# Ipsedo/MARLClassification

Hardware: AMD Instinct MI355X
Metric: agent-env-steps/sec (higher is better)
Workload: dtype f32; 1 GPU; RESISC45 256x256x3, 16 agents, 16 steps, f=12, README dims (configs[2]); full train iteration: rollout + A2C loss + BPTT backward + Adam; batch_per_gpu=256, global_batch=256, parallelism=dp1, rng=library (Philox4x32-10), launch=eager

## Files before the change

marlclassification_amd/csrc/common.h:

```cpp
#pragma once

#include <hip/hip_runtime.h>
#include <stdint.h>
#include <stdio.h>

#include "../../include/marl_hip.h"
#include "../../include/marl_hip_gemmops.h"
#include "split.h"

namespace marl {

constexpr int kWave = 64;

inline int p4(int x) { return (x + 3) & ~3; }
inline int64_t cdiv(int64_t a, int64_t b) { return (a + b - 1) / b; }

void set_error(const char* fmt, ...);

int tune_get(const char* key, int dflt);
int tune_set(const char* key, int value);

__device__ __forceinline__ float rcp_fast(float x) { return __builtin_amdgcn_rcpf(x); }
__device__ __forceinline__ float sigmoid_acc(float x) { return rcp_fast(1.0f + __expf(-x)); }
__device__ __forceinline__ float tanh_fast(float x) { return 1.0f - 2.0f * rcp_fast(1.0f + __expf(2.0f * x)); }
// ... 72 lines not shown
};

constexpr int kMaxGemmBatch = 4;
struct GemmBatch {
    GemmProb p[kMaxGemmBatch];
    int count;
    int gx, gy;
    int xcd_map;
    int single_buf;
#ifdef MARL_KERNEL_TS
    long long* ts;
#endif
};

__device__ __forceinline__ void xcd_tile(unsigned gx, unsigned gy, unsigned gz, unsigned& bx,
                                         unsigned& by, unsigned& bz) {
    const unsigned T = gx * gy * gz, L = blockIdx.x;
    const unsigned per = T >> 3, rem = T & 7, xcd = L & 7, slot = L >> 3;
    const unsigned q = (xcd < rem ? xcd * (per + 1) : rem * (per + 1) + (xcd - rem) * per) + slot;
    bz = q / (gx * gy);
    const unsigned r = q - bz * gx * gy;
    bx = r / gy;
    by = r - bx * gy;
}

inline hipError_t raise_lds(const void* kern, size_t bytes) {
    static const void* done[128];
    static int ndone = 0;
    for (int i = 0; i < ndone; ++i)
        if (done[i] == kern) return hipSuccess;
    const hipError_t e = hipFuncSetAttribute(kern, hipFuncAttributeMaxDynamicSharedMemorySize, (int)bytes);
    if (e == hipSuccess && ndone < 128) done[ndone++] = kern;
    return e;
}

GemmProb gemm_prob(const float* a, int lda, const GemmB& b, float* c, int ldc, int m, int n,
                   const float* bias = nullptr, int accumulate = 0);
void gemm_add_seg(GemmProb& p, const float* a, int lda, const GemmB& b);

using GemmPlan = marl_gemm_plan_info;
inline dim3 plan_grid(const GemmPlan& p) { return p.xcd_map ? dim3(p.gx * p.gy * p.gz) : dim3(p.gx, p.gy, p.gz); }
GemmPlan gemm_nt_plan(const GemmBatch& batch);
GemmPlan gemm_lstm_plan(const GemmBatch& batch);
int launch_gemm_nt(const GemmBatch& batch, hipStream_t st);
int launch_gemm_lstm(const GemmBatch& batch, hipStream_t st);

int split_mode();
constexpr int kSplitRowBytes = 80;
size_t split_image_floats(int rows, int k);
struct SplitDesc {
    const float* src;
    void* dst;
    int rows, k, ld, kt;
};
constexpr int kMaxSplitDesc = 64;
struct SplitBatch {
    SplitDesc d[kMaxSplitDesc];
    int count;
};
int launch_split_weights(const SplitBatch& b, hipStream_t st);
int launch_gemm_nt_split(const GemmBatch& batch, const GemmPlan& plan, bool lstm, hipStream_t st);
int launch_gemm_tn_split(const float* a, int lda, const float* b, int ldb, float* out, int ldo,
                         int64_t stride, int ni, int nj, int64_t rows, float* csum, const GemmPlan& plan, hipStream_t st);

struct G3Seg {
    const char* a3;
    const char* b3;
    int a_row0, b_row0;
    int steps;
};
struct G3Prob {
    G3Seg seg[2];
    int nseg;
    int m, n;
    float* c;
    int ldc;
    const float* bias;
    int accumulate;
    const float* c_prev;
    float* h_next;
    float* c_next;
    float* gates;
    int ld_state, ld_gates;
    char* h3;
    int h3_row0, h3_steps;
};
constexpr int kMaxG3 = 4;
struct G3Batch {
    G3Prob p[kMaxG3];
    int count;
    int gx, gy, xcd_map;
    int safe;
#ifdef MARL_G3_ABLATE
    long long* clk;
#endif
};
G3Prob g3_prob(const void* a3, int a_row0, const void* b3, int b_row0, int k, float* c, int ldc, int m, int n,
               const float* bias = nullptr, int accumulate = 0);
void g3_add_seg(G3Prob& p, const void* a3, int a_row0, const void* b3, int b_row0, int k);
GemmPlan g3_nt_plan(const G3Batch& batch, int variant = 0);
GemmPlan g3_lstm_plan(const G3Batch& batch, int variant = 0);
int launch_gemm_nt3(const G3Batch& batch, hipStream_t st, int variant = 0);
int launch_gemm_lstm3(const G3Batch& batch, hipStream_t st, int variant = 0);
struct G3TnArgs {
    const char* a3;
    const char* b3;
    int a_steps, b_steps;
    int a_row0, b_row0;
    float* out;
    int ldo;
    int64_t out_split_stride;
    int ni, nj;
    int64_t rows, rows_per_split;
    float* csum;
    int gx, gy, gz, safe;
    int j_first;
#ifdef MARL_G3_ABLATE
    int abl;
#endif
};
GemmPlan g3_tn_plan(int ni, int nj, int64_t rows, bool launch = true);
constexpr int kMaxTnCell = 4;
struct G3TnCell {
    G3TnArgs t[kMaxTnCell];
    int nt, n256;
    int gx, gz;
    int teams;
};
GemmPlan g3_tn_cell_plan(int ni, int nj_ih, int nj_hh, int64_t rows);
int gemm_tn3(const GemmPlan& plan, const char* a3, int ni, const char* b3, int nj, int64_t rows, float* c, int ldc,
             float* colsum, float* scratch, hipStream_t st);
int gemm_tn3_cell(const GemmPlan& plan, const char* g3, int ni, const char* u3, int nih, const char* h3, int nhh,
                  int64_t rows, float* c_ih, int ld_ih, float* c_hh, int ld_hh, float* colsum, float* scratch,
                  hipStream_t st);

struct ImgDesc {
    const float* src;
    void* dst;
    int64_t rows;
    int k, ld;
};
constexpr int kMaxImgDesc = 64;
struct ImgBatch {
    ImgDesc d[kMaxImgDesc];
    int count;
};
int launch_images(const ImgBatch& b, hipStream_t st);

constexpr int kProfClasses = 6;
void prof_before(int cls, hipStream_t st);
void prof_after(int cls, hipStream_t st);
int profile_begin(int cls, int max_launches);
int profile_end(double* total_ms, int* launches);

struct RedQueue;
GemmPlan tn_plan(int ni, int nj, int64_t rows, bool launch = true);
size_t gemm_tn_scratch_bytes(int ni, int nj, int64_t rows);
struct TnQueue;
int launch_gemm_tn(const float* a, int lda, const float* b, int ldb, float* c, int ldc, int ni,
                   int nj, int64_t rows, float* scratch, size_t scratch_bytes, hipStream_t st,
                   float* colsum_out = nullptr, RedQueue* q = nullptr, TnQueue* tq = nullptr);

struct TnBatchProb {
    const float* a;
    const float* b;
    float* out;
    float* csum;
    int64_t stride, rows, rows_per_split;
    int lda, ldb, ldo, ni, nj, gx, gy, first_block;
};
constexpr int kMaxTnBatch = 12;
struct TnBatch {
    TnBatchProb p[kMaxTnBatch];
    int count;
};
struct TnQueue {
    struct Item {
        const float* a;
        const float* b;
        float* c;
        float* colsum;
        int lda, ldb, ldc, ni, nj;
        int64_t rows;
    };
    Item it[kMaxTnBatch];
    int n = 0;
};
int launch_tn_queue(TnQueue& tq, RedQueue* q, hipStream_t st);

struct RedDesc {
    const float* part;
    int64_t stride;
    int count, n;
    float* out0;
    int split, nj, ldc;
    float* out1;
    int accumulate;
    int folds, per;
};
constexpr int kMaxRed = 40;
struct RedBatch {
    RedDesc d[kMaxRed];
    int first_block[kMaxRed + 1];
    int count;
};
struct RedQueue {
    RedBatch stage1, stage2;
    float* scratch = nullptr;
    size_t cap = 0, off = 0;
    hipStream_t st = nullptr;
    int rc = MARL_OK;
    void reset(float* s, size_t floats, hipStream_t stream);
    float* take(size_t floats, bool may_flush = true);
    void push(const float* part, int64_t stride, int count, int n, float* out0, int split, int nj,
              int ldc, float* out1, int accumulate);
    int launch_pending();
    int flush();
};
int launch_red_batch(const RedBatch& b, hipStream_t st);

int launch_ln_silu_fwd(const float* z, int ldz, const float* gamma, const float* beta, float* out,
                       int ldo, float* stats, int64_t m, int n, hipStream_t st,
                       const float* wdot = nullptr, const float* bdot = nullptr,
                       float* dot_out = nullptr);
int ln_bwd_blocks(int64_t m, int n);
int launch_ln_silu_bwd_rank(const float* g, int ldg, int kin, const float* bt, int ldbt,
                            const float* z, int ldz, const float* stats, const float* gamma,
                            const float* beta, float* dz, int lddz, float* part, int64_t m, int n,
                            hipStream_t st);
int launch_ln_silu_bwd(const float* da, int ldda, const float* z, int ldz, const float* stats,
                       const float* gamma, const float* beta, float* dz, int lddz, float* part,
                       int64_t m, int n, hipStream_t st);
int launch_reduce_affine(float* part, int64_t nparts, int n, float* dgamma, float* dbeta,
                         int accumulate, hipStream_t st, RedQueue* q = nullptr);

int gn_fwd_im2col_supported(int P, int C);
int launch_gn_silu_fwd(const float* z, const float* gamma, const float* beta, float* out,
                       int64_t ldo, int out_chw, float* stats, int64_t rows, int P, int C, int G,
                       hipStream_t st, float* cols = nullptr, int ldk = 0, int hin = 0);
int gn_bwd_blocks(int64_t rows, int C);
int launch_gn_silu_bwd(const float* da, int64_t ldda, int da_chw, const float* z,
                       const float* stats, const float* gamma, const float* beta, float* dz,
                       float* part, int64_t rows, int P, int C, int G, hipStream_t st);

int launch_agg_msg(const float* m, float* out, int ld, int na, int nb, int n, hipStream_t st);
int launch_mix_msg(const float* m, float* out, int ld, int na, int nb, int n, const float* mix, int transpose,
                   hipStream_t st);
int mix_msg_max_agents();
struct CommGate {
    const int32_t* pos;
    int radius, metric, normalize;
};
__device__ __forceinline__ bool comm_in_range(int2 p, int2 q, int radius, int metric) {
    const int dy = p.x > q.x ? p.x - q.x : q.x - p.x, dx = p.y > q.y ? p.y - q.y : q.y - p.y;
    if (metric) return (int64_t)dy * dy + (int64_t)dx * dx <= (int64_t)radius * radius;
    return (dy > dx ? dy : dx) <= radius;
}
template <int MAXA>
__device__ __forceinline__ float comm_gate_weight(const float* __restrict__ base, const CommGate& G, int na, int nb,
                                                  int b, int a, int a2) {
    const int2* __restrict__ pos = reinterpret_cast<const int2*>(G.pos);
    const int2 pa = pos[(size_t)a * nb + b];
    if (!G.normalize) {
        const int2 q = pos[(size_t)a2 * nb + b];
        const float bv = base[a * na + a2];
        return comm_in_range(pa, q, G.radius, G.metric) ? bv : 0.f;
    }
    constexpr int CH = MAXA < 8 ? MAXA : 8;
    float S = 0.f, s = 0.f, u = 0.f;
#pragma unroll
    for (int j0 = 0; j0 < MAXA; j0 += CH) {
        int2 q[CH];
        float bv[CH];
#pragma unroll
        for (int j = 0; j < CH; ++j) {
            const int jj = j0 + j < na ? j0 + j : na - 1;
            q[j] = pos[(size_t)jj * nb + b];
            bv[j] = base[a * na + jj];
        }
#pragma unroll
        for (int j = 0; j < CH; ++j) {
            if (j0 + j < na) {
                const float uj = comm_in_range(pa, q[j], G.radius, G.metric) ? bv[j] : 0.f;
                S += bv[j];
                s += uj;
                if (j0 + j == a2) u = uj;
            }
        }
    }
    return s > 0.f ? u * (S / s) : 0.f;
}
int launch_mix_msg_gated(const float* m, float* out, int ld, int na, int nb, int n, const float* mix,
                         const CommGate& gate, int transpose, hipStream_t st);
int comm_grad_blocks(int64_t pairs, int* per_out);
int comm_grad_supported(int na, int n, int n2, int ldw);
int launch_comm_grad(const float* dz, int lddz, const float* msg, int ldmsg, const float* w, int ldw, int na, int nb,
                     int steps, int n2, int n, float* part, float* out, hipStream_t st);

int launch_pos_embed_fwd(const int32_t* pos, const float* npos_in, int h, int w, const float* W, const float* b,
                         const float* gamma, const float* beta, float* npos4, float* z, int ldz,
                         float* stats, float* out, int ldo, int64_t rows, int nd, hipStream_t st);

int launch_lstm_cell_bwd(const float* dh, int lddh, float* dc, int lddc, float* gates, int ldg,
                         const float* c_prev, const float* c_new, int ldc, int64_t rows, int n,
                         hipStream_t st);
struct LstmBwdBatch;
// ... 482 lines not shown
```

marlclassification_amd/csrc/loss.hip:

```cpp
#include "common.h"

#include <cassert>
#include <type_traits>

namespace marl {

__device__ __forceinline__ float wsum(float v) {
#pragma unroll
    for (int o = 32; o > 0; o >>= 1) v += __shfl_xor(v, o);
    return v;
}
__device__ __forceinline__ float wmax(float v) {
#pragma unroll
    for (int o = 32; o > 0; o >>= 1) v = fmaxf(v, __shfl_xor(v, o));
    return v;
}

template <int K>
__device__ __forceinline__ void block_tree(double (*sh)[256], const double (&v)[K]) {
#pragma unroll
    for (int k = 0; k < K; ++k) sh[k][threadIdx.x] = v[k];
    __syncthreads();
    for (int o = 128; o > 0; o >>= 1) {
        if (threadIdx.x < o) {
// ... 276 lines not shown
                const float g = (expf(pbar[wave][c] - mx) / s * hs - qb[c]) * inv;
                for (int a = 0; a < na; ++a)
                    g_preds[((int64_t)t * R + (int64_t)a * nb + b) * ld_gp + c] = g;
            }
        }
    } else {
        __shared__ float wcls[4][1024];
        const float ls = logf(s);
        float wn = 0.f, wt = 0.f;
        float hn = 0.f, hs = 0.f;
        for (int c = lane; c < nc; c += 64) {
            const float wc = o.w ? o.w[c] : 1.0f;
            wcls[wave][c] = wc;
            const float nll = -(pbar[wave][c] - mx - ls);
            wn = fmaf(wc, nll, wn);
            wt += wc;
            const float qc = qb[c];
            if (qc == 0.f) continue;
            const float hc = o.keep * wc * qc;
            hn += hc * nll;
            hs += hc;
        }
        wn = wsum(wn);
        wt = wsum(wt);
        hn = wsum(hn);
        hs = wsum(hs);
        const float st = o.sw ? o.sw[t] : 1.0f;
        if (lane == 0) {
            float e = hn;
            if (o.eps_nc != 0.f) e = fmaf(o.eps_nc, wn, e);
            err[tb] = st * e;
        }
        if (g_preds) {
            const float sc = st * (1.0f / (float)R);
            const float qs = o.eps_nc != 0.f ? fmaf(o.eps_nc, wt, hs) : hs;
            for (int c = lane; c < nc; c += 64) {
                const float qv = qb[c];
                const float qc = (qv == 0.f ? 0.0f : o.keep * wcls[wave][c] * qv) + o.eps_nc * wcls[wave][c];
                const float g = (expf(pbar[wave][c] - mx) / s * qs - qc) * sc;
                for (int a = 0; a < na; ++a)
                    g_preds[((int64_t)t * R + (int64_t)a * nb + b) * ld_gp + c] = g;
            }
        }
    }
}

__global__ __launch_bounds__(256) void loss_returns_kernel(const float* __restrict__ rew,
                                                           const float* __restrict__ values,
                                                           float* __restrict__ ret,
                                                           float* __restrict__ adv,
                                                           double* __restrict__ part, int ns,
                                                           int64_t R, float gamma) {
    __shared__ double sh[2][256];
    const int64_t r = (int64_t)blockIdx.x * 256 + threadIdx.x;
    double s[2] = {0.0, 0.0};
    if (r < R) {
        float S = 0.f;
        for (int t = ns - 1; t >= 0; --t) {
            const float gt = powf(gamma, (float)t);
            S += rew[(int64_t)t * R + r] * gt;
            const float rt = S / gt;
            const float ad = rt - values[(int64_t)t * R + r];
            ret[(int64_t)t * R + r] = rt;
            adv[(int64_t)t * R + r] = ad;
            s[0] += (double)ad;
            s[1] += (double)ad * (double)ad;
        }
    }
    block_tree<2>(sh, s);
    if (threadIdx.x == 0) {
        part[2 * blockIdx.x] = sh[0][0];
        part[2 * blockIdx.x + 1] = sh[1][0];
    }
}

__global__ __launch_bounds__(256) void loss_stats_kernel(
    const double* __restrict__ part, int nblocks, const float* __restrict__ err, int64_t nerr,
    double* __restrict__ part_err, double* __restrict__ adv_stats, double n) {
    __shared__ double sh[3][256];
    double s[3] = {0.0, 0.0, 0.0};
    for (int i = threadIdx.x; i < nblocks; i += 256) {
        s[0] += part[2 * i];
        s[1] += part[2 * i + 1];
    }
    for (int64_t i = threadIdx.x; i < nerr; i += 256) s[2] += (double)err[i];
    block_tree<3>(sh, s);
    if (threadIdx.x == 0) {
        adv_stats[0] = n;
        adv_stats[1] = sh[0][0];
        adv_stats[2] = sh[1][0];
        part_err[0] = sh[2][0];
    }
}

template <bool ENT, bool VEC>
__global__ __launch_bounds__(256) void loss_grads_kernel(
    const float* __restrict__ logp, const float* __restrict__ values,
    const float* __restrict__ ret, const float* __restrict__ adv,
    const double* __restrict__ adv_stats, float* __restrict__ g_logp,
    float* __restrict__ g_values, double* __restrict__ part, int64_t NR, int64_t R,
    const float* __restrict__ probs, float* __restrict__ g_probs, double* __restrict__ part_ent, int nA,
    float beta) {
    constexpr int K = ENT ? 3 : 2;
    __shared__ double sh[K][256];
    const int64_t i = (int64_t)blockIdx.x * 256 + threadIdx.x;
    double s[K] = {};
    if (i < NR) {
        const float advn = standardized(adv[i], adv_stats);
        const float invR = 1.0f / (float)R;
        s[0] = (double)(-logp[i] * advn);
        float dg;
        s[1] = (double)smooth_l1(values[i] - ret[i], &dg);
        if (g_logp) g_logp[i] = -advn * invR;
        if (g_values) g_values[i] = dg * invR;
        if constexpr (ENT) s[2] = (double)(-row_entropy<VEC>(probs + i * nA, g_probs + i * nA, nA, beta * invR));
    }
    block_tree<K>(sh, s);
    if (threadIdx.x == 0) {
        part[2 * blockIdx.x] = sh[0][0];
        part[2 * blockIdx.x + 1] = sh[1][0];
        if constexpr (ENT) part_ent[blockIdx.x] = sh[2][0];
    }
}

template <bool ENT>
__global__ __launch_bounds__(256) void loss_final_kernel(
    const double* __restrict__ part, int nblocks, const double* __restrict__ part_err,
    float* __restrict__ scalars, int ns, int nb, int64_t R, const double* __restrict__ part_ent, float beta) {
    constexpr int K = ENT ? 3 : 2;
    __shared__ double sh[K][256];
    double s[K] = {};
    for (int i = threadIdx.x; i < nblocks; i += 256) {
        s[0] += part[2 * i];
        s[1] += part[2 * i + 1];
        if constexpr (ENT) s[2] += part_ent[i];
    }
    block_tree<K>(sh, s);
    if (threadIdx.x == 0) {
        const double path = sh[0][0] / (double)R, critic = sh[1][0] / (double)R;
        const double esum = part_err[0];
        double loss = path + esum / (double)nb + critic;
        if constexpr (ENT) {
            const double h = sh[2][0];
            loss -= (double)beta * (h / (double)R);
            scalars[4] = (float)(h / ((double)R * ns));
        }
        scalars[0] = (float)loss;
        scalars[1] = (float)path;
        scalars[2] = (float)(esum / ((double)ns * nb));
        scalars[3] = (float)critic;
    }
}

static ClassOpt class_opt(const LossCommon& a) {
    return ClassOpt{a.cls_w, a.cls_sw, 1.0f - a.cls_eps, a.cls_eps / (float)a.nc};
}

static void launch_rewards(const LossCommon& a, float* rew, hipStream_t st) {
    const int64_t NR = (int64_t)a.na * a.nb * a.ns;
    const float rnd = (float)log((double)a.nc);
    if (a.soft_q) {
        if (a.cls && a.cls_wrew && a.cls_w)
            hipLaunchKernelGGL(loss_rewards_soft_kernel<true>, dim3((unsigned)cdiv(NR, 4)), dim3(256), 0, st, a.preds,
                               a.soft_q, rew, NR, a.nb, a.nc, rnd, class_opt(a));
        else
            hipLaunchKernelGGL(loss_rewards_soft_kernel<false>, dim3((unsigned)cdiv(NR, 4)), dim3(256), 0, st, a.preds,
                               a.soft_q, rew, NR, a.nb, a.nc, rnd, NoClassOpt{});
        return;
    }
    if (a.cls && a.cls_wrew && a.cls_w)
        hipLaunchKernelGGL(loss_rewards_kernel<true>, dim3((unsigned)cdiv(NR, 4)), dim3(256), 0, st, a.preds, a.y, rew,
                           NR, a.nb, a.nc, rnd, class_opt(a));
    else
        hipLaunchKernelGGL(loss_rewards_kernel<false>, dim3((unsigned)cdiv(NR, 4)), dim3(256), 0, st, a.preds, a.y,
                           rew, NR, a.nb, a.nc, rnd, NoClassOpt{});
}

static void launch_error(const LossGradArgs& a, float* err, hipStream_t st) {
    const dim3 grid((unsigned)cdiv((int64_t)a.ns * a.nb, 4));
    if (a.soft_q) {
        if (a.cls)
            hipLaunchKernelGGL(loss_error_soft_kernel<true>, grid, dim3(256), 0, st, a.preds, a.soft_q, err, a.g_preds,
                               a.ld_gp, a.ns, a.na, a.nb, a.nc, class_opt(a));
        else
            hipLaunchKernelGGL(loss_error_soft_kernel<false>, grid, dim3(256), 0, st, a.preds, a.soft_q, err, a.g_preds,
                               a.ld_gp, a.ns, a.na, a.nb, a.nc, NoClassOpt{});
        return;
    }
    if (a.cls)
        hipLaunchKernelGGL(loss_error_kernel<true>, grid, dim3(256), 0, st, a.preds, a.y, err, a.g_preds, a.ld_gp, a.ns,
                           a.na, a.nb, a.nc, class_opt(a));
    else
        hipLaunchKernelGGL(loss_error_kernel<false>, grid, dim3(256), 0, st, a.preds, a.y, err, a.g_preds, a.ld_gp,
                           a.ns, a.na, a.nb, a.nc, NoClassOpt{});
}

int launch_loss(const LossArgs& a, hipStream_t st) {
    if (a.nc > 1024) {
        set_error("nb_class %d > 1024 unsupported by the loss kernel", a.nc);
        return MARL_ELIMIT;
    }
    const int64_t R = (int64_t)a.na * a.nb, NR = R * a.ns;
    LossLayout L = loss_layout(a.scratch, a.ns, a.na, a.nb);
    double* stats = reinterpret_cast<double*>(a.adv_stats);
    if (a.phase == 0 || a.phase == 1) {
        launch_rewards(a, L.rew, st);
        MARL_LAUNCH_CHECK();
        launch_error(a, L.err, st);
        MARL_LAUNCH_CHECK();
        hipLaunchKernelGGL(loss_returns_kernel, dim3((unsigned)L.blocksC), dim3(256), 0, st, L.rew,
                           a.values, L.ret, L.adv, L.part_adv, a.ns, R, a.gamma);
        MARL_LAUNCH_CHECK();
        hipLaunchKernelGGL(loss_stats_kernel, dim3(1), dim3(256), 0, st, L.part_adv, L.blocksC,
                           L.err, (int64_t)a.ns * a.nb, L.part_err, stats, (double)NR);
        MARL_LAUNCH_CHECK();
    }
    if (a.phase == 0 || a.phase == 2) {
        double* part_ent = extra_partials(L, 1);
        with_grads_instance(a, [&](auto ent, auto vec) {
            hipLaunchKernelGGL((loss_grads_kernel<decltype(ent)::value, decltype(vec)::value>), dim3((unsigned)L.blocksE),
                               dim3(256), 0, st, a.logp, a.values, L.ret, L.adv, stats, a.g_logp, a.g_values,
                               L.part_loss, NR, R, a.probs, a.g_probs, part_ent, a.n_act, a.entropy_coef);
        });
        MARL_LAUNCH_CHECK();
        if (a.probs)
            hipLaunchKernelGGL(loss_final_kernel<true>, dim3(1), dim3(256), 0, st, L.part_loss, L.blocksE, L.part_err,
                               a.scalars, a.ns, a.nb, R, part_ent, a.entropy_coef);
        else
            hipLaunchKernelGGL(loss_final_kernel<false>, dim3(1), dim3(256), 0, st, L.part_loss, L.blocksE, L.part_err,
                               a.scalars, a.ns, a.nb, R, nullptr, 0.f);
        MARL_LAUNCH_CHECK();
    }
    return MARL_OK;
}


__global__ __launch_bounds__(256) void loss_gae_kernel(const float* __restrict__ rew,
                                                       const float* __restrict__ values,
                                                       float* __restrict__ ret, float* __restrict__ adv,
                                                       double* __restrict__ part, int ns, int64_t R,
                                                       float gamma, float lam) {
    __shared__ double sh[2][256];
    const int64_t r = (int64_t)blockIdx.x * 256 + threadIdx.x;
    double s[2] = {0.0, 0.0};
    if (r < R) {
        const float gl = gamma * lam;
        float A = 0.f, vnext = 0.f;
        for (int t = ns - 1; t >= 0; --t) {
            const int64_t i = (int64_t)t * R + r;
            const float v = values[i];
            const float delta = rew[i] + gamma * vnext - v;
            A = delta + gl * A;
            vnext = v;
            ret[i] = A + v;
            adv[i] = A;
            s[0] += (double)A;
            s[1] += (double)A * (double)A;
        }
    }
    block_tree<2>(sh, s);
    if (threadIdx.x == 0) {
        part[2 * blockIdx.x] = sh[0][0];
        part[2 * blockIdx.x + 1] = sh[1][0];
    }
}

__global__ __launch_bounds__(256) void loss_standardize_kernel(const float* __restrict__ adv,
                                                               const double* __restrict__ adv_stats,
                                                               float* __restrict__ advn, int64_t NR) {
    const int64_t i = (int64_t)blockIdx.x * 256 + threadIdx.x;
    if (i >= NR) return;
    advn[i] = standardized(adv[i], adv_stats);
}

int launch_advantages(const AdvArgs& a, hipStream_t st) {
    const int64_t R = (int64_t)a.na * a.nb, NR = R * a.ns;
    LossLayout L = loss_layout(a.scratch, a.ns, a.na, a.nb);
    double* stats = reinterpret_cast<double*>(a.adv_stats);
    if (a.phase == 0 || a.phase == 1) {
        launch_rewards(a, L.rew, st);
        MARL_LAUNCH_CHECK();
        if (a.lam == 1.0f)
            hipLaunchKernelGGL(loss_returns_kernel, dim3((unsigned)L.blocksC), dim3(256), 0, st, L.rew, a.values,
                               a.ret, L.adv, L.part_adv, a.ns, R, a.gamma);
        else
            hipLaunchKernelGGL(loss_gae_kernel, dim3((unsigned)L.blocksC), dim3(256), 0, st, L.rew, a.values, a.ret,
                               L.adv, L.part_adv, a.ns, R, a.gamma, a.lam);
        MARL_LAUNCH_CHECK();
        hipLaunchKernelGGL(loss_stats_kernel, dim3(1), dim3(256), 0, st, L.part_adv, L.blocksC, L.err, (int64_t)0,
                           L.part_err, stats, (double)NR);
        MARL_LAUNCH_CHECK();
    }
    if (a.phase == 0 || a.phase == 2) {
        hipLaunchKernelGGL(loss_standardize_kernel, dim3((unsigned)L.blocksE), dim3(256), 0, st, L.adv, stats,
                           a.advn, NR);
        MARL_LAUNCH_CHECK();
    }
    return MARL_OK;
}

template <bool ENT, bool VEC>
__global__ __launch_bounds__(256) void ppo_grads_kernel(
    const float* __restrict__ logp, const float* __restrict__ old_logp, const float* __restrict__ values,
    const float* __restrict__ ret, const float* __restrict__ advn_in, float clip_eps, float* __restrict__ g_logp,
    float* __restrict__ g_values, double* __restrict__ part, double* __restrict__ extra, int64_t NR, int64_t R,
    const float* __restrict__ probs, float* __restrict__ g_probs, int nA, float beta) {
    __shared__ double sh[5][256];
    const int64_t i = (int64_t)blockIdx.x * 256 + threadIdx.x;
    double s[5] = {0.0, 0.0, 0.0, 0.0, 0.0};
    if (i < NR) {
        const float advn = advn_in[i];
        const float invR = 1.0f / (float)R;
        const float lp = logp[i], olp = old_logp[i];
        const float rho = expf(lp - olp);
        const float lo = 1.0f - clip_eps, hi = 1.0f + clip_eps;
        const bool clipped = (advn > 0.f && rho > hi) || (advn < 0.f && rho < lo);
        const float rc = fminf(fmaxf(rho, lo), hi);
        s[0] = (double)(-(clipped ? rc : rho) * advn);
        float dg;
        s[1] = (double)smooth_l1(values[i] - ret[i], &dg);
        s[3] = (double)(olp - lp);
        s[4] = clipped ? 1.0 : 0.0;
        if (g_logp) g_logp[i] = clipped ? 0.f : (-advn * rho) * invR;
        if (g_values) g_values[i] = dg * invR;
        if (ENT) s[2] = (double)(-row_entropy<VEC>(probs + i * nA, g_probs + i * nA, nA, beta * invR));
    }
    block_tree<5>(sh, s);
    if (threadIdx.x == 0) {
        part[2 * blockIdx.x] = sh[0][0];
        part[2 * blockIdx.x + 1] = sh[1][0];
        extra[3 * blockIdx.x] = sh[2][0];
        extra[3 * blockIdx.x + 1] = sh[3][0];
        extra[3 * blockIdx.x + 2] = sh[4][0];
    }
}

__global__ __launch_bounds__(256) void ppo_final_kernel(const double* __restrict__ part,
                                                        const double* __restrict__ extra, int nblocks,
                                                        const float* __restrict__ err, int64_t nerr,
                                                        float* __restrict__ scalars, int ns, int nb, int64_t R,
                                                        float beta) {
    __shared__ double sh[6][256];
    double s[6] = {0.0, 0.0, 0.0, 0.0, 0.0, 0.0};
    for (int i = threadIdx.x; i < nblocks; i += 256) {
        s[0] += part[2 * i];
        s[1] += part[2 * i + 1];
        s[2] += extra[3 * i];
        s[3] += extra[3 * i + 1];
        s[4] += extra[3 * i + 2];
    }
    for (int64_t i = threadIdx.x; i < nerr; i += 256) s[5] += (double)err[i];
    block_tree<6>(sh, s);
    if (threadIdx.x == 0) {
        const double NR = (double)R * ns;
        const double surr = sh[0][0] / (double)R, critic = sh[1][0] / (double)R, h = sh[2][0];
        const double esum = sh[5][0];
        scalars[0] = (float)(surr + esum / (double)nb + critic - (double)beta * (h / (double)R));
// ... 103 lines not shown
```

marlclassification_amd/csrc/rowops.hip:

```cpp
#include <stdarg.h>

#include <ctype.h>
#include <stdlib.h>
#include <string.h>

#include "common.h"
#include "sample.h"

namespace marl {

static thread_local char g_err[512] = "";
void set_error(const char* fmt, ...) {
    va_list ap;
    va_start(ap, fmt);
    vsnprintf(g_err, sizeof(g_err), fmt, ap);
    va_end(ap);
}
const char* last_error() { return g_err; }

namespace {
struct Knob {
    char key[32];
    int value;
    bool set;
};
constexpr int kMaxKnobs = 128;
Knob g_knobs[kMaxKnobs];
int g_nknobs = 0;
Knob* knob(const char* key, bool create) {
    for (int i = 0; i < g_nknobs; ++i)
        if (!strcmp(g_knobs[i].key, key)) return &g_knobs[i];
    if (!create || g_nknobs >= kMaxKnobs || strlen(key) >= sizeof(g_knobs[0].key)) return nullptr;
    Knob* k = &g_knobs[g_nknobs++];
    strcpy(k->key, key);
    k->value = 0;
    k->set = false;
    return k;
}
}

static const char* const kKnownKnobs[] = {
    "g3", "g3_lstm", "g3_tn", "g3_min_units", "g3_safe", "mfma_split", "g3_lstm_variant", "g3_nt_variant",
    "g3_tn_variant", "g3_tn_cell", "g3_tn_pipe", "g3_tn_wgs", "nt_xcd", "tn_xcd", "panel_chain", "red_defer",
    "tn_split_waves", "wgrad3", "cnn_fwd2", "cnn_fwd3", "dgrad_wgs", "dgrad_min_chunks",
    "g3_clk", "g3_tn_abl",
};

int tune_set(const char* key, int value) {
    bool known = false;
    for (const char* name : kKnownKnobs) known = known || !strcmp(name, key);
    if (!known) {
        set_error("marl_tune: unknown knob %s", key);
        return MARL_EINVAL;
    }
    Knob* k = knob(key, true);
    if (!k) {
        set_error("marl_tune: knob table full or key too long (%s)", key);
        return MARL_EINVAL;
    }
    k->value = value;
    k->set = true;
    return MARL_OK;
}

int tune_get(const char* key, int dflt) {
    Knob* k = knob(key, true);
    if (k && k->set) return k->value;
    char env[48] = "MARL_";
    size_t n = strlen(env);
    for (const char* c = key; *c && n + 1 < sizeof(env); ++c) env[n++] = (char)toupper((unsigned char)*c);
    env[n] = 0;
    const char* e = getenv(env);
    const int v = e ? atoi(e) : dflt;
    if (k && e) {
        k->value = v;
        k->set = true;
    }
    return v;
}

__device__ __forceinline__ float wave_max(float v) {
#pragma unroll
    for (int o = 32; o > 0; o >>= 1) v = fmaxf(v, __shfl_xor(v, o));
    return v;
}
__device__ __forceinline__ float silu_f(float y) { return silu_fast(y); }
__device__ __forceinline__ float silu_grad(float y) { return silu_grad_fast(y); }

__global__ __launch_bounds__(256) void ln_silu_fwd_kernel(const float* __restrict__ z, int ldz,
                                                          const float* __restrict__ gamma,
                                                          const float* __restrict__ beta,
                                                          float* __restrict__ out, int ldo,
                                                          float* __restrict__ stats, int64_t m,
                                                          int n) {
    const int lane = threadIdx.x & 63;
    const int64_t row = (int64_t)blockIdx.x * 4 + (threadIdx.x >> 6);
    if (row >= m) return;
    const float* zr = z + row * ldz;
    float s = 0.f;
    for (int c = lane; c < n; c += 64) s += zr[c];
    const float mean = wave_sum(s) / (float)n;
    float q = 0.f;
    for (int c = lane; c < n; c += 64) {
        const float d = zr[c] - mean;
        q += d * d;
    }
    const float rstd = 1.0f / sqrtf(wave_sum(q) / (float)n + 1e-5f);
    float* orow = out + row * ldo;
    for (int c = lane; c < n; c += 64) {
        const float y = (zr[c] - mean) * rstd * gamma[c] + beta[c];
        orow[c] = silu_f(y);
    }
    if (stats && lane == 0) {
        stats[row * 2] = mean;
        stats[row * 2 + 1] = rstd;
    }
}

template <int U>
__global__ __launch_bounds__(256) void ln_silu_fwd_reg_kernel(const float* __restrict__ z, int ldz,
                                                              const float* __restrict__ gamma,
                                                              const float* __restrict__ beta,
                                                              float* __restrict__ out, int ldo,
                                                              float* __restrict__ stats, int64_t m,
                                                              int n, const float* __restrict__ wdot,
                                                              const float* __restrict__ bdot,
                                                              float* __restrict__ dot_out, int64_t half) {
    const int lane = threadIdx.x & 63;
    const int64_t row0 = (int64_t)blockIdx.x * 4 + (threadIdx.x >> 6);
    if (row0 >= half) return;
    const int64_t rows[2] = {row0, row0 + half};
    const bool ok1 = rows[1] < m;
    float v[2][U], gm[U], bt[U], wd[U];
#pragma unroll
    for (int u = 0; u < U; ++u) {
        const int c = lane + 64 * u;
        v[0][u] = c < n ? z[rows[0] * ldz + c] : 0.f;
        v[1][u] = (c < n && ok1) ? z[rows[1] * ldz + c] : 0.f;
        gm[u] = c < n ? gamma[c] : 0.f;
        bt[u] = c < n ? beta[c] : 0.f;
        wd[u] = (c < n && wdot) ? wdot[c] : 0.f;
    }
#pragma unroll
    for (int k = 0; k < 2; ++k) {
        if (k == 1 && !ok1) break;
        const int64_t row = rows[k];
        float s = 0.f;
#pragma unroll
        for (int u = 0; u < U; ++u) s += v[k][u];
        const float mean = wave_sum(s) / (float)n;
        float q = 0.f;
#pragma unroll
        for (int u = 0; u < U; ++u) {
            const float d = (lane + 64 * u < n) ? v[k][u] - mean : 0.f;
            v[k][u] = d;
            q += d * d;
        }
        const float rstd = 1.0f / sqrtf(wave_sum(q) / (float)n + 1e-5f);
        float* orow = out + row * ldo;
        float dot = 0.f;
#pragma unroll
        for (int u = 0; u < U; ++u) {
            const int c = lane + 64 * u;
            if (c < n) {
                const float a = silu_f(v[k][u] * rstd * gm[u] + bt[u]);
                orow[c] = a;
                dot += a * wd[u];
            }
        }
        if (stats && lane == 0) {
            stats[row * 2] = mean;
            stats[row * 2 + 1] = rstd;
        }
        if (wdot) {
            dot = wave_sum(dot);
            if (lane == 0) dot_out[row] = dot + bdot[0];
        }
    }
}

int launch_ln_silu_fwd(const float* z, int ldz, const float* gamma, const float* beta, float* out,
                       int ldo, float* stats, int64_t m, int n, hipStream_t st, const float* wdot,
                       const float* bdot, float* dot_out) {
    if (m <= 0) return MARL_OK;
    const int64_t half = (m + 1) / 2;
    dim3 grid((unsigned)cdiv(n <= 384 ? half : m, 4)), blk(256);
    if (wdot && n > 384) {
        set_error("fused row dot needs a LayerNorm width <= 384");
        return MARL_ELIMIT;
    }
    if (n <= 128)
        hipLaunchKernelGGL(ln_silu_fwd_reg_kernel<2>, grid, blk, 0, st, z, ldz, gamma, beta, out, ldo,
                           stats, m, n, wdot, bdot, dot_out, half);
    else if (n <= 384)
        hipLaunchKernelGGL(ln_silu_fwd_reg_kernel<6>, grid, blk, 0, st, z, ldz, gamma, beta, out, ldo,
                           stats, m, n, wdot, bdot, dot_out, half);
    else
        hipLaunchKernelGGL(ln_silu_fwd_kernel, grid, blk, 0, st, z, ldz, gamma, beta, out, ldo, stats,
                           m, n);
    MARL_LAUNCH_CHECK();
    return MARL_OK;
}

static int bwd_waves(int n) { return n <= 512 ? 16 : (n <= 1024 ? 8 : 4); }
static int bwd_rows_per_wave(int64_t m, int waves) {
    int64_t r = cdiv(m, (int64_t)waves * 256);
    if (r < 1) r = 1;
    if (r > 64) r = 64;
    return (int)r;
}
int ln_bwd_blocks(int64_t m, int n) {
    const int w = bwd_waves(n);
    return (int)cdiv(m, (int64_t)w * bwd_rows_per_wave(m, w));
}

__global__ __launch_bounds__(1024) void ln_silu_bwd_kernel(
    const float* __restrict__ da, int ldda, const float* __restrict__ z, int ldz,
    const float* __restrict__ stats, const float* __restrict__ gamma,
    const float* __restrict__ beta, float* __restrict__ dz, int lddz, float* __restrict__ part,
    int64_t m, int n, int rpw) {
    extern __shared__ __attribute__((aligned(16))) float sacc[];
    const int lane = threadIdx.x & 63;
    const int wave = threadIdx.x >> 6;
    const int nwaves = blockDim.x >> 6;
    float* ga = sacc + (size_t)wave * 2 * n;
    float* gb = ga + n;
    for (int c = lane; c < n; c += 64) {
        ga[c] = 0.f;
        gb[c] = 0.f;
    }
    for (int rr = 0; rr < rpw; ++rr) {
// ... 1765 lines not shown
```

Baseline: 9.798 million agent-env-steps/s.

## Fuse loss rewards/error and stats/grads/finalize kernels into fewer launches

Adds a fused kernel that computes per-agent rewards and the averaged-vote classification error (plus its gradient) in one pass, and a second kernel that folds the advantage stats reduction, per-element gradients and final scalar reduction together, using a ticket counter so the last block finishes the loss. The phase-0 loss path drops from about five or more launches to three when no soft targets, class options or entropy are in use, cutting launch overhead in eager mode. In exchange, every block recomputes the global stats reduction redundantly, and the ticket lives in scratch just past the error buffer, which depends on the layout leaving room there. An environment variable can turn the merged path off.

```diff
diff --git a/marlclassification_amd/csrc/common.h b/marlclassification_amd/csrc/common.h
--- a/marlclassification_amd/csrc/common.h
+++ b/marlclassification_amd/csrc/common.h
@@ -248,6 +248,8 @@
 void prof_after(int cls, hipStream_t st);
 int profile_begin(int cls, int max_launches);
 int profile_end(double* total_ms, int* launches);
+
+bool small_launches_merged();
 
 struct RedQueue;
 GemmPlan tn_plan(int ni, int nj, int64_t rows, bool launch = true);
diff --git a/marlclassification_amd/csrc/loss.hip b/marlclassification_amd/csrc/loss.hip
--- a/marlclassification_amd/csrc/loss.hip
+++ b/marlclassification_amd/csrc/loss.hip
@@ -452,6 +452,152 @@
     }
 }
 
+
+template <int CPL, int ROWS>
+__global__ __launch_bounds__(256) void loss_rewards_error_kernel(const float* __restrict__ preds,
+                                                                 const int64_t* __restrict__ y,
+                                                                 float* __restrict__ rew, float* __restrict__ err,
+                                                                 float* __restrict__ g_preds, int ld_gp, int ns, int na,
+                                                                 int nb, int nc, float rnd,
+                                                                 unsigned int* __restrict__ ticket) {
+    __shared__ float pbar[4][64 * CPL];
+    const int lane = threadIdx.x & 63, wave = threadIdx.x >> 6;
+    if (blockIdx.x == 0 && threadIdx.x == 0) *ticket = 0u;
+    const int64_t tb = (int64_t)blockIdx.x * 4 + wave;
+    if (tb >= (int64_t)ns * nb) return;
+    const int t = (int)(tb / nb), b = (int)(tb % nb);
+    const int64_t R = (int64_t)na * nb;
+    const int yb = (int)y[b];
+    float vote[CPL];
+#pragma unroll
+    for (int k = 0; k < CPL; ++k) vote[k] = 0.f;
+    for (int a0 = 0; a0 < na; a0 += ROWS) {
+        float v[ROWS][CPL];
+#pragma unroll
+        for (int u = 0; u < ROWS; ++u) {
+            const int a = a0 + u < na ? a0 + u : na - 1;
+            const float* p = preds + ((int64_t)t * R + (int64_t)a * nb + b) * nc;
+#pragma unroll
+            for (int k = 0; k < CPL; ++k) v[u][k] = lane + 64 * k < nc ? p[lane + 64 * k] : 0.f;
+        }
+#pragma unroll
+        for (int u = 0; u < ROWS; ++u) {
+            if (a0 + u >= na) break;
+            const int64_t row = (int64_t)t * R + (int64_t)(a0 + u) * nb + b;
+            float mx = -INFINITY;
+#pragma unroll
+            for (int k = 0; k < CPL; ++k)
+                if (lane + 64 * k < nc) mx = fmaxf(mx, v[u][k]);
+            mx = wmax(mx);
+            float s = 0.f;
+#pragma unroll
+            for (int k = 0; k < CPL; ++k)
+                if (lane + 64 * k < nc) s += expf(v[u][k] - mx);
+            s = wsum(s);
+            if (lane == 0) {
+                const float ce = -(preds[row * nc + yb] - mx - logf(s));
+                rew[row] = (rnd - ce) / rnd;
+            }
+#pragma unroll
+            for (int k = 0; k < CPL; ++k) vote[k] += v[u][k];
+        }
+    }
+    float mx = -INFINITY;
+#pragma unroll
+    for (int k = 0; k < CPL; ++k) {
+        const int c = lane + 64 * k;
+        if (c < nc) {
+            const float s = vote[k] / (float)na;
+            pbar[wave][c] = s;
+            mx = fmaxf(mx, s);
+        }
+    }
+    mx = wmax(mx);
+    float s = 0.f;
+    for (int c = lane; c < nc; c += 64) s += expf(pbar[wave][c] - mx);
+    s = wsum(s);
+    if (lane == 0) err[tb] = -(pbar[wave][yb] - mx - logf(s));
+    if (g_preds) {
+        const float inv = 1.0f / (float)R;
+        for (int c = lane; c < nc; c += 64) {
+            const float g = (expf(pbar[wave][c] - mx) / s - (c == yb ? 1.0f : 0.0f)) * inv;
+            for (int a = 0; a < na; ++a)
+                g_preds[((int64_t)t * R + (int64_t)a * nb + b) * ld_gp + c] = g;
+        }
+    }
+}
+
+__device__ __forceinline__ float standardized_by(float adv, double n, double sum, double sumsq) {
+    const double mean_d = sum / n;
+    const double var_d = (sumsq - sum * mean_d) / (n - 1.0);
+    const float mean = (float)mean_d;
+    const float sd = (float)sqrt(var_d > 0.0 ? var_d : 0.0);
+    return (adv - mean) / (sd + 1e-8f);
+}
+
+__global__ __launch_bounds__(256) void loss_grads_final_kernel(
+    const double* __restrict__ part_adv, int nblocks_adv, const float* __restrict__ err, int64_t nerr,
+    double* __restrict__ part_err, double* __restrict__ adv_stats, double n, const float* __restrict__ logp,
+    const float* __restrict__ values, const float* __restrict__ ret, const float* __restrict__ adv,
+    float* __restrict__ g_logp, float* __restrict__ g_values, double* part, int64_t NR, int64_t R,
+    float* __restrict__ scalars, int ns, int nb, unsigned int* ticket) {
+    __shared__ double sh[3][256];
+    __shared__ bool last;
+    double st[3] = {0.0, 0.0, 0.0};
+    for (int i = threadIdx.x; i < nblocks_adv; i += 256) {
+        st[0] += part_adv[2 * i];
+        st[1] += part_adv[2 * i + 1];
+    }
+    for (int64_t i = threadIdx.x; i < nerr; i += 256) st[2] += (double)err[i];
+    block_tree<3>(sh, st);
+    const double sum = sh[0][0], sumsq = sh[1][0], esum = sh[2][0];
+    if (blockIdx.x == 0 && threadIdx.x == 0) {
+        adv_stats[0] = n;
+        adv_stats[1] = sum;
+        adv_stats[2] = sumsq;
+        part_err[0] = esum;
+    }
+    __syncthreads();
+
+    const int64_t i = (int64_t)blockIdx.x * 256 + threadIdx.x;
+    double s[2] = {};
+    if (i < NR) {
+        const float advn = standardized_by(adv[i], n, sum, sumsq);
+        const float invR = 1.0f / (float)R;
+        s[0] = (double)(-logp[i] * advn);
+        float dg;
+        s[1] = (double)smooth_l1(values[i] - ret[i], &dg);
+        if (g_logp) g_logp[i] = -advn * invR;
+        if (g_values) g_values[i] = dg * invR;
+    }
+    block_tree<2>(sh, s);
+    if (threadIdx.x == 0) {
+        __hip_atomic_store(&part[2 * blockIdx.x], sh[0][0], __ATOMIC_RELAXED, __HIP_MEMORY_SCOPE_AGENT);
+        __hip_atomic_store(&part[2 * blockIdx.x + 1], sh[1][0], __ATOMIC_RELAXED, __HIP_MEMORY_SCOPE_AGENT);
+        const unsigned int drawn = __hip_atomic_fetch_add(ticket, 1u, __ATOMIC_ACQ_REL, __HIP_MEMORY_SCOPE_AGENT);
+        last = drawn == gridDim.x - 1;
+    }
+    __syncthreads();
+    if (!last) return;
+
+    const int nblocks = (int)gridDim.x;
+    double f[2] = {};
+    for (int j = threadIdx.x; j < nblocks; j += 256) {
+        f[0] += __hip_atomic_load(&part[2 * j], __ATOMIC_RELAXED, __HIP_MEMORY_SCOPE_AGENT);
+        f[1] += __hip_atomic_load(&part[2 * j + 1], __ATOMIC_RELAXED, __HIP_MEMORY_SCOPE_AGENT);
+    }
+    block_tree<2>(sh, f);
+    if (threadIdx.x == 0) {
+        const double path = sh[0][0] / (double)R, critic = sh[1][0] / (double)R;
+        const double loss = path + esum / (double)nb + critic;
+        scalars[0] = (float)loss;
+        scalars[1] = (float)path;
+        scalars[2] = (float)(esum / ((double)ns * nb));
+        scalars[3] = (float)critic;
+        __hip_atomic_store(ticket, 0u, __ATOMIC_RELAXED, __HIP_MEMORY_SCOPE_AGENT);
+    }
+}
+
 static ClassOpt class_opt(const LossCommon& a) {
     return ClassOpt{a.cls_w, a.cls_sw, 1.0f - a.cls_eps, a.cls_eps / (float)a.nc};
 }
@@ -503,6 +649,26 @@
     const int64_t R = (int64_t)a.na * a.nb, NR = R * a.ns;
     LossLayout L = loss_layout(a.scratch, a.ns, a.na, a.nb);
     double* stats = reinterpret_cast<double*>(a.adv_stats);
+    if (a.phase == 0 && !a.soft_q && !a.cls && !a.probs && small_launches_merged()) {
+        unsigned int* ticket = reinterpret_cast<unsigned int*>(L.err + (int64_t)a.ns * a.nb + 15);
+        const float rnd = (float)log((double)a.nc);
+        const dim3 grid((unsigned)cdiv((int64_t)a.ns * a.nb, 4));
+        if (a.nc <= 64)
+            hipLaunchKernelGGL((loss_rewards_error_kernel<1, 8>), grid, dim3(256), 0, st, a.preds, a.y, L.rew, L.err,
+                               a.g_preds, a.ld_gp, a.ns, a.na, a.nb, a.nc, rnd, ticket);
+        else
+            hipLaunchKernelGGL((loss_rewards_error_kernel<16, 1>), grid, dim3(256), 0, st, a.preds, a.y, L.rew, L.err,
+                               a.g_preds, a.ld_gp, a.ns, a.na, a.nb, a.nc, rnd, ticket);
+        MARL_LAUNCH_CHECK();
+        hipLaunchKernelGGL(loss_returns_kernel, dim3((unsigned)L.blocksC), dim3(256), 0, st, L.rew,
+                           a.values, L.ret, L.adv, L.part_adv, a.ns, R, a.gamma);
+        MARL_LAUNCH_CHECK();
+        hipLaunchKernelGGL(loss_grads_final_kernel, dim3((unsigned)L.blocksE), dim3(256), 0, st, L.part_adv, L.blocksC,
+                           L.err, (int64_t)a.ns * a.nb, L.part_err, stats, (double)NR, a.logp, a.values, L.ret, L.adv,
+                           a.g_logp, a.g_values, L.part_loss, NR, R, a.scalars, a.ns, a.nb, ticket);
+        MARL_LAUNCH_CHECK();
+        return MARL_OK;
+    }
     if (a.phase == 0 || a.phase == 1) {
         launch_rewards(a, L.rew, st);
         MARL_LAUNCH_CHECK();
diff --git a/marlclassification_amd/csrc/rowops.hip b/marlclassification_amd/csrc/rowops.hip
--- a/marlclassification_amd/csrc/rowops.hip
+++ b/marlclassification_amd/csrc/rowops.hip
@@ -77,6 +77,14 @@
         k->set = true;
     }
     return v;
+}
+
+bool small_launches_merged() {
+    static const bool on = [] {
+        const char* v = getenv("MARL_SMALL_LAUNCHES");
+        return !(v && v[0] == '1');
+    }();
+    return on;
 }
 
 __device__ __forceinline__ float wave_max(float v) {
```

Result: no change. 9.824 million agent-env-steps/s (median of 6 runs) (+0.3%).
